# fpgasystems/GPU-FPGA-Recommendation-System

Measured on AMD Instinct MI355X. Metric: inferences/sec at batch 256, higher is better.
Workload: dtype f32; 1 GPU; Model-A (embedding_47_krnl: 47 tables, 1.415 GB) batch=256, fp32 FC 352-1024-512-256-1, all tables resident in one GPU's HBM; hash-filled tables, uniform per-table indices; index rows resident in HBM when the timed region starts (1024 rotating buffers), scores left in HBM (the bench contract's definition of `value`); value_pcie_inclusive = the reference's own loop (cuda_server.c:460-461,494-495): ; batch=256, driver_threads=2, workers_per_thread=2, batches_per_launch=64, parallelism=replicas x1

## Files before the change

gpu-fpga-recommendation-system_amd/csrc/fr_api.cpp:

```cpp
#include <chrono>
#include <cmath>
#include <cstdarg>
#include <cstdio>
#include <cstdlib>
#include <cstring>
#include <new>

#include "fr_internal.h"

static thread_local char g_err[512] = "";

void fr_set_error(const char *fmt, ...) {
    va_list ap;
    va_start(ap, fmt);
    vsnprintf(g_err, sizeof(g_err), fmt, ap);
    va_end(ap);
}

#ifdef FR_EXPERIMENTS
int fr_knob_env(const char *name, int dflt) {
    const char *e = getenv(name);
    return e ? atoi(e) : dflt;
}
#endif
// ... 718 lines not shown
    if (w->ctx) (void)hipSetDevice(w->ctx->device);
    fr_comm_worker_release(w);
    if (w->stream) (void)hipStreamSynchronize(w->stream);
    if (w->counted) w->ctx->n_workers.fetch_sub(1, std::memory_order_relaxed);
    if (w->h_idx) (void)hipHostFree(w->h_idx);
    if (w->h_pool_w) (void)hipHostFree(w->h_pool_w);
    if (w->h_pool_off) (void)hipHostFree(w->h_pool_off);
    if (w->h_dense) (void)hipHostFree(w->h_dense);
    if (w->h_score) (void)hipHostFree(w->h_score);
    if (w->h_err) (void)hipHostFree(w->h_err);
    if (w->h_sh_status) (void)hipHostFree(w->h_sh_status);
    if (w->h_stage_send) (void)hipHostFree(w->h_stage_send);
    if (w->h_stage_recv) (void)hipHostFree(w->h_stage_recv);
    void *dev[] = {w->d_idx, w->d_dense, w->d_records, w->d_act[0], w->d_act[1], w->d_score, w->d_slice, w->d_gathered, w->d_score_part, w->d_score_all};
    for (void *p : dev)
        if (p) (void)hipFree(p);
    if (w->hr.h_idx) (void)hipHostFree(w->hr.h_idx);
    if (w->hr.h_dense) (void)hipHostFree(w->hr.h_dense);
    if (w->hr.h_sc) (void)hipHostFree(w->hr.h_sc);
    void *hdev[] = {w->hr.d_idx, w->hr.d_dense, w->hr.d_sc};
    for (void *p : hdev)
        if (p) (void)hipFree(p);
    for (hipEvent_t e : w->hr.ev)
        if (e) (void)hipEventDestroy(e);
    for (hipEvent_t e : w->hr.ev_in)
        if (e) (void)hipEventDestroy(e);
    if (w->hr.copy) {
        (void)hipStreamSynchronize(w->hr.copy);
        (void)hipStreamDestroy(w->hr.copy);
    }
    if (w->h_blist) (void)hipHostFree(w->h_blist);
    if (w->d_blist) (void)hipFree(w->d_blist);
    for (hipEvent_t e : w->ev_blist)
        if (e) (void)hipEventDestroy(e);
    if (w->ev_update) (void)hipEventDestroy(w->ev_update);
    if (w->ev_start) (void)hipEventDestroy(w->ev_start);
    if (w->ev_stop) (void)hipEventDestroy(w->ev_stop);
    if (w->stream) (void)hipStreamDestroy(w->stream);
    fr_ctx *held = w->counted ? w->ctx : nullptr;
    delete w;
    fr_ctx_unref(held);
}

static size_t idx_cols(const fr_ctx *c) {
    const int mode = c->model.index_mode;
    return mode == FR_INDEX_PER_TABLE ? (size_t)c->model.n_tables : (mode == FR_INDEX_PER_BANK ? (size_t)c->n_banks : 1);
}

#define W_HIP(call)                                                                       \
    do {                                                                                  \
        hipError_t e_ = (call);                                                           \
        if (e_ != hipSuccess) {                                                           \
            fr_set_error("%s failed: %s", #call, hipGetErrorString(e_));                  \
            fr_worker_destroy(w);                                                         \
            return (e_ == hipErrorOutOfMemory) ? FR_ERR_OOM : FR_ERR_HIP;                 \
        }                                                                                 \
    } while (0)

extern "C" int fr_worker_create(fr_ctx *ctx, int max_batch, fr_worker **out) {
    if (!ctx || !out) FR_FAIL(FR_ERR_INVALID, "NULL argument");
    *out = nullptr;
    if (max_batch <= 0 || max_batch > (1 << 24)) FR_FAIL(FR_ERR_INVALID, "max_batch %d out of range", max_batch);
    {
        int widest = 0;
        for (int l = 0; l < 4; l++) widest = ctx->model.fc[l] > widest ? ctx->model.fc[l] : widest;
        if ((uint64_t)widest * (uint64_t)round_up(max_batch, 64) * 4ull >= (1ull << 32))
// ... 520 lines not shown
extern "C" int fr_ctx_set_small_block(fr_ctx *ctx, int max_batches) {
    if (!ctx) FR_FAIL(FR_ERR_INVALID, "ctx is NULL");
    if (max_batches < 0 || max_batches > 8) FR_FAIL(FR_ERR_INVALID, "max_batches %d outside [0, 8]", max_batches);
    ctx->small_block.store(max_batches, std::memory_order_relaxed);
    return FR_OK;
}

extern "C" int fr_ctx_stream_group(const fr_ctx *ctx) { return (ctx && !ctx->cpu && fused_eligible(ctx)) ? fused_group(ctx) : 1; }

static int fused_launch_slice(fr_worker *w, FrFusedArgs &a, int first, int n) {
    fr_ctx *c = w->ctx;
    const bool bf16 = c->fc_precision == FR_FC_BF16, fp8 = c->fc_precision == FR_FC_FP8;
    const int m2_forced = FR_KNOB_ONCE("FUSED_M2", -1);
    int tiles64 = 0;
    for (int i = 0; i < n; i++) tiles64 += (w->pending[first + i].batch + 63) / 64;
    const bool m2 = !bf16 && c->fc_precision == FR_FC_FP32 && frk_fused_m2_ok(c->model.fc[0], c->model.fc[1], c->model.fc[2], c->model.fc[3]) &&
                    (m2_forced == 1 || (m2_forced != 0 && fused_group(c) >= 64 && tiles64 > 128));
    const int per_wg = (bf16 || fp8) ? frk_fused_h_items_per_wg() : (m2 ? 64 : 32);
    int max_tiles = 0;
    for (int i = 0; i < n; i++) {
        a.b[i] = w->pending[first + i];
        const int tiles = (a.b[i].batch + per_wg - 1) / per_wg;
        if (tiles > max_tiles) max_tiles = tiles;
    }
    a.n_batches = n;
    a.tiles_per_batch = max_tiles;
    a.blist = nullptr;
    if (fp8) return frk_fused_f8_launch(a, w->stream);
    if (m2) return frk_fused_m2_launch(a, w->stream);
    if (bf16) return frk_fused_h_launch(a, w->stream);
    return frk_fused_launch(a, w->stream);
}

static int fused_flush(fr_worker *w) {
    if (w->n_pending == 0) return FR_OK;
    fr_ctx *c = w->ctx;
    FrFusedArgs a{};
    const bool bf16 = c->fc_precision == FR_FC_BF16, fp8 = c->fc_precision == FR_FC_FP8;
    a.words = c->d_words;
    a.n_words = c->n_words;
    a.idx_stride = (int)idx_cols(c);
    a.err_flag = w->d_err;
    if (fp8) {
        a.w1q = reinterpret_cast<const float4 *>(c->d_w_fp8[0]);
        a.w2q = reinterpret_cast<const float4 *>(c->d_w_fp8[1]);
        a.w3q = reinterpret_cast<const float4 *>(c->d_w_fp8[2]);
        a.wout = c->d_w[3];
        for (int l = 0; l < 3; l++) a.e_w[l] = c->f8_e_w[l];
        for (int l = 0; l < 4; l++) a.e_act[l] = c->f8_e_act[l];
    } else if (bf16) {
        a.w1q = reinterpret_cast<const float4 *>(c->d_w_bf16[0]);
        a.w2q = reinterpret_cast<const float4 *>(c->d_w_bf16[1]);
        a.w3q = reinterpret_cast<const float4 *>(c->d_w_bf16[2]);
        a.wout = reinterpret_cast<const float *>(c->d_w_bf16[3]);
    } else {
        a.w1q = reinterpret_cast<const float4 *>(c->d_wq[0]);
        a.w2q = reinterpret_cast<const float4 *>(c->d_wq[1]);
        a.w3q = reinterpret_cast<const float4 *>(c->d_wq[2]);
        a.wout = c->d_w[3];
    }
    a.K = c->model.fc[0];
    a.H1 = c->model.fc[1];
    a.H2 = c->model.fc[2];
    a.H3 = c->model.fc[3];
    a.stamps = g_stamp_buffer;
    const int n_all = w->n_pending;
    w->n_pending = 0;
    w->pending_items = 0;
    struct Keep {
        fr_worker *w;
        ~Keep() { keep_kernel(w); }
    } keep{w};
    if (bf16 || (fp8 && FR_KNOB_ONCE("FUSED_HK", -1) == 1 && c->d_w_fp8h[0] && c->d_w_fp8h[1] && c->d_w_fp8h[2])) {
        int tiles = 0, max_tiles = 0;
        for (int i = 0; i < n_all; i++) {
            const int t_ = (w->pending[i].batch + 63) / 64;
            tiles += t_;
            if (t_ > max_tiles) max_tiles = t_;
        }
        const int hk = FR_KNOB_ONCE("FUSED_HK", -1);
        const int hs_from = a.K <= 352 ? c->n_cu : c->n_cu + c->n_cu / 4;
        const bool only_hs = bf16 && !frk_fused_h_ok(a.K, a.H1, a.H2, a.H3);
        if (c->hk_ok == 1 && (only_hs || (hk != 0 && (hk == 1 || tiles >= hs_from)))) {
            if (!w->h_blist) {
                FR_HIP(hipHostMalloc((void **)&w->h_blist, sizeof(FrFusedBatch) * FR_FUSED_MAX_QUEUE * FR_BLIST_RING, hipHostMallocDefault));
                FR_HIP(hipMalloc((void **)&w->d_blist, sizeof(FrFusedBatch) * FR_FUSED_MAX_QUEUE * FR_BLIST_RING));
                for (int k = 0; k < FR_BLIST_RING; k++) FR_HIP(hipEventCreateWithFlags(&w->ev_blist[k], hipEventDisableTiming));
            }
            const int k = w->blist_cur;
            w->blist_cur = (k + 1) % FR_BLIST_RING;
            if (w->blist_busy[k]) FR_HIP(hipEventSynchronize(w->ev_blist[k]));
            FrFusedBatch *hb = w->h_blist + (size_t)k * FR_FUSED_MAX_QUEUE, *db = w->d_blist + (size_t)k * FR_FUSED_MAX_QUEUE;
            memcpy(hb, w->pending, sizeof(FrFusedBatch) * n_all);
            FR_HIP(hipMemcpyAsync(db, hb, sizeof(FrFusedBatch) * n_all, hipMemcpyHostToDevice, w->stream));
            FR_HIP(hipEventRecord(w->ev_blist[k], w->stream));
            w->blist_busy[k] = true;
            a.blist = db;
            a.n_batches = n_all;
            a.tiles_per_batch = max_tiles;
            if (bf16 && frk_fused_hk_takes_lp_rows(a.K) && lp_image_applies_hs(c)) {
                const int irc = lp_ensure_image(c, FR_FC_BF16);
                if (irc) return irc;
                a.words = c->d_words_lp;
                a.src_lp = 1;
            }
            if (bf16 && FR_KNOB_ONCE("FUSED_HS_ABLATE", 0)) a.e_act[3] = -776 - FR_KNOB_ONCE("FUSED_HS_ABLATE", 0);
            if (fp8) {
                a.w1q = reinterpret_cast<const float4 *>(c->d_w_fp8h[0]);
                a.w2q = reinterpret_cast<const float4 *>(c->d_w_fp8h[1]);
                a.w3q = reinterpret_cast<const float4 *>(c->d_w_fp8h[2]);
            }
            return frk_fused_hk_launch(a, c->n_cu, c->fc_precision, w->stream);
        }
    }
    for (int first = 0; first < n_all; first += FR_FUSED_MAX_BATCHES) {
        const int n = n_all - first < FR_FUSED_MAX_BATCHES ? n_all - first : FR_FUSED_MAX_BATCHES;
        int rc = fused_launch_slice(w, a, first, n);
        if (rc) return rc;
    }
    return FR_OK;
}

static int check_gather_args(fr_worker *w, const int32_t *d_idx, const float *d_dense) {
    fr_ctx *c = w->ctx;
    if (!d_idx) FR_FAIL(FR_ERR_INVALID, "d_idx is NULL");
    if (c->model.dense_len && !d_dense) FR_FAIL(FR_ERR_INVALID, "model has dense features but d_dense is NULL");
    return FR_OK;
}

static int launch_fc(fr_worker *w, int batch, const float *d_records, float *d_scores) {
    fr_ctx *c = w->ctx;
    if (c->n_shards > 1) FR_FAIL(FR_ERR_STATE, "fc on a sharded ctx needs the all-gathered records (use the sharded driver: fr_worker_submit_sharded, fr_worker_submit_sharded_pooled)");
    if (c->cpu) {
        frc_fc_chain(c->model.fc, c->d_w, d_records, batch, w->c_scratch, d_scores);
        return FR_OK;
    }
    if (w->n_active) FR_FAIL(FR_ERR_STATE, "pipeline busy: call fr_worker_sync first");
    if (w->launch_no == 0) w->launch_no = 1;
    const int ldm = round_up(batch, 32);
    const int par_prev = (int)((w->launch_no - 1) & 1);
    int rc;
    if (c->fc_precision == FR_FC_FP8) rc = frk_records_to_q16_fp8(d_records, act_set(w, par_prev).x, batch, c->model.fc[0], ldm, c->f8_e_act[0], w->stream);
    else if (c->fc_precision == FR_FC_BF16) rc = frk_records_to_q8_bf16(d_records, act_set(w, par_prev).x, batch, c->model.fc[0], ldm, w->stream);
    else rc = frk_transpose_records(d_records, act_set(w, par_prev).x, batch, c->model.fc[0], ldm, w->stream);
    if (rc) return rc;
    rc = pipeline_push(w, batch, 1, nullptr, nullptr, d_scores);
    if (rc) return rc;
    return pipeline_flush(w);
}

static int fc_from_slices_impl(fr_worker *w, int batch_total, int item0, int n_items, const float *d_gathered, float *d_scores, uint64_t *stage1_launch) {
    int rc = check_ready(w, n_items, false, true);
    if (rc) return rc;
// ... 464 lines not shown
    if (rc) return rc;
    if (!d_scores) FR_FAIL(FR_ERR_INVALID, "d_scores is NULL");
    fr_ctx *c = w->ctx;
    if (c->n_shards > 1 || c->model.layout != FR_LAYOUT_SEMANTIC)
        FR_FAIL(FR_ERR_STATE, "push_device needs an unsharded SEMANTIC-layout context");
    rc = check_gather_args(w, d_idx, d_dense);
    if (rc) return rc;
    if (c->cpu) {
        rc = launch_pipeline(w, batch, d_idx, d_dense, d_scores);
        if (rc) return rc;
        w->in_flight = true;
        return FR_OK;
    }
    FR_SET_DEVICE(c);
    const bool idx_fits = (size_t)batch * idx_cols(c) * sizeof(int32_t) < ((size_t)4000 << 20);
    const bool fused = fused_eligible(c) && fused_group(c) >= FR_FUSED_MIN_GROUP && idx_fits;
    if (fused && w->n_active > 0) {
        rc = pipeline_flush(w);
        if (rc) return rc;
    }
    if (!fused && w->n_pending > 0) {
        rc = fused_flush(w);
        if (rc) return rc;
    }
    if (fused) {
        FrFusedBatch &fb = w->pending[w->n_pending++];
        fb.idx = d_idx;
        fb.dense = d_dense;
        fb.scores = d_scores;
        fb.batch = batch;
        w->pending_items += batch;
        w->in_flight = true;
        const bool big = c->fc_precision == FR_FC_BF16 || (c->fc_precision == FR_FC_FP8 && FR_KNOB_ONCE("FUSED_HK", -1) == 1);
        const int64_t max_items = FR_KNOB_ONCE("FUSED_ITEMS", 0) ? FR_KNOB_ONCE("FUSED_ITEMS", 0) : (big ? 4096 * 64 : 256 * 64);
        return (w->n_pending >= fused_group(c) || w->pending_items >= max_items || w->n_pending >= FR_FUSED_MAX_QUEUE) ? fused_flush(w) : FR_OK;
    }
    rc = pipeline_push(w, batch, 0, d_idx, d_dense, d_scores);
    if (rc) return rc;
    w->in_flight = true;
    return FR_OK;
}

extern "C" int fr_worker_push_device_list(fr_worker *w, int n, const int *batch, const int32_t *const *d_idx, const float *const *d_dense,
                                          float *const *d_scores) {
    if (!w) FR_FAIL(FR_ERR_INVALID, "worker is NULL");
    if (n < 0 || (n > 0 && (!batch || !d_idx || !d_scores))) FR_FAIL(FR_ERR_INVALID, "push_device_list: n = %d needs batch, d_idx and d_scores arrays", n);
    for (int i = 0; i < n; i++) {
        const int rc = fr_worker_push_device(w, batch[i], d_idx[i], d_dense ? d_dense[i] : nullptr, d_scores[i]);
        if (rc) return rc;
    }
    return FR_OK;
}

static int push_pooled_impl(fr_worker *w, int batch, const int32_t *d_idx, const float *d_weights, const float *d_dense, float *d_scores, const int32_t *d_offsets = nullptr,
                            int64_t nnz = 0) {
    int rc = check_ready(w, batch, true, true);
    if (rc) return rc;
    if (!d_scores) FR_FAIL(FR_ERR_INVALID, "d_scores is NULL");
    fr_ctx *c = w->ctx;
    const bool weighted = d_weights != nullptr;
    if (c->pool_cols <= 0)
        FR_FAIL(FR_ERR_STATE, c->n_shards > 1 ? "no pooling is set on the sharded context: create it with fr_ctx_create_sharded_pooled" : "no pooling is set on the context: call fr_ctx_set_pooling first");
    if (c->n_shards > 1) FR_FAIL(FR_ERR_STATE, "a pooled push on a sharded ctx: the chain needs the all-gathered slices (fr_worker_submit_sharded_pooled)");
    if (c->model.layout != FR_LAYOUT_SEMANTIC) FR_FAIL(FR_ERR_STATE, "a pooled push needs a SEMANTIC-layout context");
    if (c->cpu) {
        rc = submit_pooled_impl(w, batch, d_idx, d_weights, weighted, d_dense, d_scores, d_offsets, nnz);
        if (rc) return rc;
        w->in_flight = true;
// ... 613 lines not shown
```

gpu-fpga-recommendation-system_amd/csrc/fr_fused.hip:

```cpp
#include "fr_device.h"

constexpr int FR_FT_LD = 33;

template <int NT, int D>
__device__ __forceinline__ void ft_load_a(float4 (&r)[D][NT], const float4 *__restrict__ aq, int N, int g) {
#pragma unroll
    for (int i = 0; i < D; i++)
#pragma unroll
        for (int t = 0; t < NT; t++) r[i][t] = aq[(size_t)(2 * (g + i)) * N + 32 * t];
}

template <int NT, int D>
__device__ __forceinline__ void ft_compute(f32x16 (&acc)[NT], f32x16 &alt, const float4 (&r)[D][NT], const uint4 *bl, int gb) {
    uint4 rb[D];
#pragma unroll
    for (int i = 0; i < D; i++) rb[i] = bl[(size_t)(2 * (gb + i)) * FR_FT_LD];
    __builtin_amdgcn_sched_barrier(0);
#pragma unroll
    for (int i = 0; i < D; i++) {
        const float bx = __uint_as_float(rb[i].x), by = __uint_as_float(rb[i].y), bz = __uint_as_float(rb[i].z), bw = __uint_as_float(rb[i].w);
        if constexpr (NT == 1) {
            acc[0] = __builtin_amdgcn_mfma_f32_32x32x2f32(r[i][0].x, bx, acc[0], 0, 0, 0);
            alt = __builtin_amdgcn_mfma_f32_32x32x2f32(r[i][0].y, by, alt, 0, 0, 0);
            acc[0] = __builtin_amdgcn_mfma_f32_32x32x2f32(r[i][0].z, bz, acc[0], 0, 0, 0);
// ... 394 lines not shown
    for (int g = 0; g < CNT; g++) {
        uint4 bnext[MT];
        const int gn = (g + 1 < CNT) ? g + 1 : g;
#pragma unroll
        for (int mt = 0; mt < MT; mt++) bnext[mt] = bl[(size_t)(2 * gn) * FR_M2_LD + 32 * mt];
        const float4(&a4)[NT] = ring[g % R];
#pragma unroll
        for (int c = 0; c < 4; c++)
#pragma unroll
            for (int t = 0; t < NT; t++)
#pragma unroll
                for (int mt = 0; mt < MT; mt++) {
                    const float av = c == 0 ? a4[t].x : c == 1 ? a4[t].y : c == 2 ? a4[t].z : a4[t].w;
                    const uint32_t bv = c == 0 ? bcur[mt].x : c == 1 ? bcur[mt].y : c == 2 ? bcur[mt].z : bcur[mt].w;
                    if (NT == 1 && (c & 1)) alt[mt] = __builtin_amdgcn_mfma_f32_32x32x2f32(av, __uint_as_float(bv), alt[mt], 0, 0, 0);
                    else acc[t][mt] = __builtin_amdgcn_mfma_f32_32x32x2f32(av, __uint_as_float(bv), acc[t][mt], 0, 0, 0);
                }
        if (g + R < CNT) {
#pragma unroll
            for (int t = 0; t < NT; t++) ring[g % R][t] = ft_wload(w, s0 + (unsigned)(g + R) * w.row2, 512 * t);
        }
        __builtin_amdgcn_sched_barrier(0);
#pragma unroll
        for (int mt = 0; mt < MT; mt++) bcur[mt] = bnext[mt];
    }
    if constexpr (NT == 1) {
#pragma unroll
        for (int mt = 0; mt < MT; mt++)
#pragma unroll
            for (int i = 0; i < 16; i++) acc[0][mt][i] += alt[mt][i];
    }
}

__device__ __forceinline__ void ftm_store_tile(uint4 *img, const f32x16 &acc, int n_local, int m_local, int hk, int lm) {
#pragma unroll
    for (int i = 0; i < 4; i++) {
        uint4 v;
        v.x = __float_as_uint(acc[4 * i + 0]);
        v.y = __float_as_uint(acc[4 * i + 1]);
        v.z = __float_as_uint(acc[4 * i + 2]);
        v.w = __float_as_uint(acc[4 * i + 3]);
        img[(size_t)((n_local >> 2) + 2 * i + hk) * FR_M2_LD + m_local + lm] = v;
    }
}

template <int KG>
__global__ void __launch_bounds__(512) fr_fused_tile_m2_kernel(const FrFusedArgs a) {
    extern __shared__ uint4 lds[];
    constexpr int LD = FR_M2_LD, MT = 2, T2W = 2, TI = 64;
    constexpr int RA = 12, RB = 8;
    const int KQ = a.K / 4;
    uint4 *Xq = lds;
    uint4 *R1 = Xq + (size_t)KQ * LD;
    uint4 *R2 = lds;
    uint4 *R3 = lds;
    const int tid = threadIdx.x, lane = tid & 63;
    const int wave = __builtin_amdgcn_readfirstlane(tid >> 6);
    const int hk = lane >> 5, lm = lane & 31;
    const int bi = blockIdx.x / a.tiles_per_batch, tile = blockIdx.x - bi * a.tiles_per_batch;
    const FrFusedBatch &bt = a.b[bi];
    const int m0 = tile * TI;
    if (m0 >= bt.batch) return;
    const FtW W1 = ft_w(a.w1q, a.K, a.H1, hk, lm), W2 = ft_w(a.w2q, a.H1, a.H2, hk, lm), W3 = ft_w(a.w3q, a.H2, a.H3, hk, lm);
    float4 ring1[RA][1];
    ft_ring_fill<1, RA, KG>(ring1, W1, 32 * wave, 0);

    {
        const int wl = tid & 63, ig = tid >> 6;
        constexpr int NB = (2 * KG + 63) / 64;
        const bool bad = ft_gather_tile<NB, 8>(a, bt, m0, wl, ig, [&](int w, int i, const uint4 &x) { Xq[(size_t)w * LD + 8 * ig + i] = x; });
        if (bad) atomicOr_system(a.err_flag, 1);
    }
    __syncthreads();

    f32x16 acc2[T2W][MT];
#pragma unroll
    for (int t = 0; t < T2W; t++)
#pragma unroll
        for (int mt = 0; mt < MT; mt++)
#pragma unroll
            for (int i = 0; i < 16; i++) acc2[t][mt][i] = 0.0f;
// ... 32 lines not shown
    ftm_gemm_ct<1, MT, RA, 32 * T2W>(acc3, ring3, W3, 32 * wave, R2, 0, 0, hk, lm);
    __syncthreads();
#pragma unroll
    for (int mt = 0; mt < MT; mt++) ftm_store_tile(R3, acc3[0][mt], 32 * wave, 32 * mt, hk, lm);
    __syncthreads();
    {
        const int il = tid & 63, sg = tid >> 6;
        const int rows_per = (a.H3 / 4) / 16;
        float *part = reinterpret_cast<float *>(R3 + (size_t)(a.H3 / 4) * LD);
#pragma unroll
        for (int h2 = 0; h2 < 2; h2++) {
            const int sl = 2 * sg + h2;
            float s = 0.0f;
            for (int q = sl * rows_per; q < (sl + 1) * rows_per; q++) {
                const uint4 r = R3[(size_t)q * LD + il];
                const float4 w4 = reinterpret_cast<const float4 *>(a.wout)[q];
                s = fmaf(w4.x, __uint_as_float(r.x), s);
                s = fmaf(w4.y, __uint_as_float(r.y), s);
                s = fmaf(w4.z, __uint_as_float(r.z), s);
                s = fmaf(w4.w, __uint_as_float(r.w), s);
            }
            part[sl * 64 + il] = s;
        }
        __syncthreads();
        if (tid < 64 && m0 + tid < bt.batch) {
            float t = part[tid];
#pragma unroll
            for (int i = 1; i < 16; i++) t += part[i * 64 + tid];
            bt.scores[m0 + tid] = t;
        }
    }
}

bool frk_fused_m2_ok(int K, int H1, int H2, int H3) { return K == 352 && H1 % 256 == 0 && H2 == 512 && H3 == 256; }

int frk_fused_m2_launch(const FrFusedArgs &a, hipStream_t s) {
    static FrLdsAttrOnce lds_once;
    if (int rc_ = fr_allow_full_lds(&fr_fused_tile_m2_kernel<44>, lds_once)) return rc_;
    const size_t rows1 = (size_t)(a.K / 4) + 64, rows2 = (size_t)(a.H2 / 4), rows3 = 64 + 4;
    const size_t rows = rows1 > rows2 ? (rows1 > rows3 ? rows1 : rows3) : (rows2 > rows3 ? rows2 : rows3);
    fr_fused_tile_m2_kernel<44><<<dim3(a.n_batches * a.tiles_per_batch), dim3(512), rows * FR_M2_LD * 16, s>>>(a);
    fr_note_kernel("fr_fused_tile_m2_kernel<44>");
    KCHECK();
    return FR_OK;
}

template <int NT, int MT, int R, int CNT>
__device__ __forceinline__ void fth_gemm_ct(f32x16 (&acc)[NT][MT], const FtW &w, int n0, const uint4 *Bh, int ld, int gb0, int g0, int hk, int lm) {
    const unsigned s0 = (unsigned)g0 * w.row2 + (unsigned)n0 * 16u;
    const uint4 *bl = Bh + (size_t)(2 * gb0 + hk) * ld + lm;
    uint4 ring[R][NT];
#pragma unroll
    for (int g = 0; g < R && g < CNT; g++)
#pragma unroll
        for (int t = 0; t < NT; t++) ring[g][t] = __builtin_bit_cast(uint4, ft_wload(w, s0 + (unsigned)g * w.row2, 512 * t));
#pragma unroll
    for (int g = 0; g < CNT; g++) {
        uint4 b8[MT];
#pragma unroll
        for (int mt = 0; mt < MT; mt++) b8[mt] = bl[(size_t)(2 * g) * ld + 32 * mt];
#pragma unroll
        for (int t = 0; t < NT; t++)
#pragma unroll
            for (int mt = 0; mt < MT; mt++)
                acc[t][mt] = __builtin_amdgcn_mfma_f32_32x32x16_bf16(__builtin_bit_cast(bf16x8, ring[g % R][t]), __builtin_bit_cast(bf16x8, b8[mt]),
                                                                     acc[t][mt], 0, 0, 0);
        if (g + R < CNT) {
#pragma unroll
            for (int t = 0; t < NT; t++) ring[g % R][t] = __builtin_bit_cast(uint4, ft_wload(w, s0 + (unsigned)(g + R) * w.row2, 512 * t));
        }
        __builtin_amdgcn_sched_barrier(0);
    }
}

// ... 406 lines not shown
```

gpu-fpga-recommendation-system_amd/csrc/fr_internal.h:

```cpp
#pragma once

#include <hip/hip_runtime.h>

#include <atomic>
#include <mutex>
#include <cstdint>
#include <string>
#include <vector>

#include "fleetrec.h"
#include "fleetrec_diag.h"
#include "fleetrec_serving.h"

void fr_set_error(const char *fmt, ...) __attribute__((format(printf, 1, 2)));

#define FR_FAIL(code, ...)         \
    do {                           \
        fr_set_error(__VA_ARGS__); \
        return (code);             \
    } while (0)

#define FR_HIP(call)                                                                                 \
    do {                                                                                             \
        hipError_t e_ = (call);                                                                      \
// ... 229 lines not shown
    int c_err = 0;
    double c_t0 = 0.0;
    hipStream_t stream = nullptr;
    int32_t *h_idx = nullptr;
    float *h_dense = nullptr;
    float *h_score = nullptr;
    int32_t *d_idx = nullptr;
    float *d_dense = nullptr;
    float *d_records = nullptr;
    float *d_act[2] = {nullptr, nullptr};
    int ld_max = 0;
    struct Slot {
        bool active = false;
        uint64_t launch0 = 0;
        int first_stage = 0;
        int batch = 0, ldm = 0;
        const int32_t *d_idx = nullptr;
        const float *d_dense = nullptr;
        float *d_scores = nullptr;
    } ring[8];
    uint64_t launch_no = 0;
    int n_active = 0;
    bool counted = false;
    bool diag_launch = false;
    bool calibrating = false;
    int last_x_parity = 0;
    FrFusedBatch pending[FR_FUSED_MAX_QUEUE];
    int n_pending = 0;
    FrFusedBatch *h_blist = nullptr, *d_blist = nullptr;
    hipEvent_t ev_blist[FR_BLIST_RING] = {nullptr, nullptr, nullptr, nullptr};
    bool blist_busy[FR_BLIST_RING] = {false, false, false, false};
    int blist_cur = 0;
    int64_t pending_items = 0;
    float *d_score = nullptr;
    struct HostRing {
        int g = 0;
        size_t idx_slot = 0, dense_slot = 0, score_slot = 0;
        int32_t *h_idx = nullptr, *d_idx = nullptr;
        float *h_dense = nullptr, *d_dense = nullptr, *h_sc = nullptr, *d_sc = nullptr;
        hipEvent_t ev[4] = {nullptr, nullptr, nullptr, nullptr};
        hipStream_t copy = nullptr;
        hipEvent_t ev_in[4] = {nullptr, nullptr, nullptr, nullptr};
        bool inflight[4] = {false, false, false, false};
        int count[4] = {0, 0, 0, 0};
        float *dst[4][FR_FUSED_MAX_BATCHES];
        int bsz[4][FR_FUSED_MAX_BATCHES];
        int cur = 0;
        int staged = 0;
        long long delivered = 0;
    } hr;
    void *d_slice = nullptr, *d_gathered = nullptr;
    float *d_score_part = nullptr, *d_score_all = nullptr;
    float *h_sh_status = nullptr;
    struct fr_comm *sh_comm = nullptr;
    int sh_ranks = 0;
    std::atomic<int> sh_inject_fc_fail{0};
    void *h_stage_send = nullptr, *h_stage_recv = nullptr;
    void *sh_host_stream = nullptr;
    int *h_err = nullptr;
    int *d_err = nullptr;
    bool in_flight = false;
    hipEvent_t ev_update = nullptr;
    bool update_recorded = false;
    char last_kernel[96] = "";
    hipEvent_t ev_start = nullptr, ev_stop = nullptr;
};
// ... 35 lines not shown
int frk_scatter_rows(float *head, int64_t row_stride_bytes, float *tail, int64_t head_rows, int64_t rows, int dim, int n, const int32_t *ids, const float *src, int *err_flag,
                     hipStream_t s);
int frk_gather(const FrWordDesc *words, int n_words, const FrGatherGroups &groups, const int32_t *idx, int idx_stride, const float *dense, void *out, int batch, int *err_flag,
               int transport, int e_x, hipStream_t s, int out_words, bool one_chunk = false);
int frk_gather_pooled(const FrWordDesc *words, const FrPoolDesc *pool, int n_words, const FrGatherGroups &groups, const int32_t *idx, const float *weights, int pool_cols,
                      int max_hots, bool wide, bool any_mean, const float *dense, void *out, int batch, int *err_flag, hipStream_t s, int out_words,
                      const int32_t *offsets = nullptr, int n_icols = 0, long long nnz = 0, int operand = 0, int ldm = 0, int e_x = 0, bool item_major = false);
int frk_gather_tile(const FrPassDesc *passes, const FrChunkDesc *chunks, int n_chunks, const int32_t *idx, int idx_stride, const float *dense, void *out,
                    int out_stride_words, int batch, int *err_flag, bool dedup, unsigned long long *dup_counter, hipStream_t s);
int frk_transpose_slices_lp(int precision, const void *gathered, int n_shards, int batch_total, int slice_padded, const int *h_offsets, const int *h_lens,
                            int item0, int n_items, void *X, int K, int ldm, hipStream_t s);
int frk_pipeline_launch(const FrPipeArgs &a, int single_stage, int precision, hipStream_t s);
int frk_pack_weights_q8_bf16(const float *W, uint16_t *Wh, int K, int H, hipStream_t s);
bool frk_fc_lp_gemm_ok(int precision, int K, int N, int ldm);
int frk_fc_lp_gemm(int precision, const void *Wp, const void *Xp, void *Yp, int K, int N, int ldm, int e_w, int e_in, int e_out, int width, bool minor, hipStream_t s);
bool frk_fused_hk_takes_lp_rows(int K);
bool frk_fc_tail_ok(int precision, int K, int N, int ldm);
int frk_fc_tail(int precision, const void *W3, const void *R2, const void *wout, float *scores, int K, int N, int ldm, int batch, int e_w, int e_in, int e_r3, hipStream_t s);
int frk_records_to_q8_bf16(const float *X, void *Xh, int batch, int K, int ldm, hipStream_t s);
int frk_pack_weights_q16_fp8(const float *W, void *Wf, int K, int H, int e_w, hipStream_t s);
int frk_pack_weights_q16h_fp8(const float *W, void *Wg, int K, int H, int e_w, hipStream_t s);
int frk_records_to_q16_fp8(const float *X, void *Xf, int batch, int K, int ldm, int e_x, hipStream_t s);
int frk_stats(const float *p, size_t n, void *d_out, hipStream_t s);
int frk_q4_to_lp(int precision, const float *Xq, void *Xo, int K, int ldm, int e_x, hipStream_t s);
int frk_stage_blocks_f8_gather(int K, int ldm);
int frk_pack_weights_q4(const float *W, float *Wq, int K, int H, hipStream_t s);
int frk_stage_blocks(int stage, int n_words, int K, int N, int ldm, int nsplit);
int frk_gather_tr_blocks(int n_words, int ldm, int variant);
int frk_gather_tr_variant(int batch, int idx_stride);
bool frk_fused_ok(int K, int H1, int H2, int H3);
int frk_fused_launch(const FrFusedArgs &a, hipStream_t s);
bool frk_fused_m2_ok(int K, int H1, int H2, int H3);
int frk_fused_m2_launch(const FrFusedArgs &a, hipStream_t s);
bool frk_fused_h_ok(int K, int H1, int H2, int H3);
bool frk_fused_f8_ok(int K, int H1, int H2, int H3);
int frk_fused_f8_launch(const FrFusedArgs &a, hipStream_t s);
int frk_fused_h_items_per_wg();
int frk_fused_h_launch(const FrFusedArgs &a, hipStream_t s);
bool frk_fused_hk_ok(int K, int H1, int H2, int H3, const FrWordDesc *h_words, int n_words);
int frk_fused_hk_launch(const FrFusedArgs &a, int n_cu, int precision, hipStream_t s);
int frk_transpose_records(const float *X, float *Xt, int batch, int K, int ldm, hipStream_t s);
int frk_transpose_slices(const float *gathered, int n_shards, int batch_total, int slice_padded, const int *h_offsets, const int *h_lens,
                         int item0, int n_items, float *Xq, int ldm, hipStream_t s);
void fr_shard_bounds(const fr_model_desc &m, int n_shards, std::vector<int> &seg_begin);
int fr_bank_map(const fr_model_desc &m, std::vector<int> &bank_of_table, std::vector<int64_t> &bank_min_rows);
```

Baseline: 69.31 million inferences/s.

## Add persistent fp32 fused MLP kernel overlapping next-tile gather with layer-3 GEMM

Adds a persistent variant of the fp32 m2 fused kernel that launches one workgroup per CU and loops over tiles taken from a device-resident batch list. Inside the layer-3 GEMM it issues the descriptor, index and embedding-row loads for the next tile through scheduling hooks, so gather latency hides behind MFMA work. The host side now holds pushes to enlarge launches, flushes only whole CU fills when it can, and uses events to detect a launch backlog. This removes per-tile workgroup launch and gather-stall costs, in exchange for more complex flush logic, extra latency from held batches and higher register pressure.

```diff
diff --git a/gpu-fpga-recommendation-system_amd/csrc/fr_api.cpp b/gpu-fpga-recommendation-system_amd/csrc/fr_api.cpp
--- a/gpu-fpga-recommendation-system_amd/csrc/fr_api.cpp
+++ b/gpu-fpga-recommendation-system_amd/csrc/fr_api.cpp
@@ -774,6 +774,8 @@
     if (w->h_blist) (void)hipHostFree(w->h_blist);
     if (w->d_blist) (void)hipFree(w->d_blist);
     for (hipEvent_t e : w->ev_blist)
+        if (e) (void)hipEventDestroy(e);
+    for (hipEvent_t e : w->ev_fused)
         if (e) (void)hipEventDestroy(e);
     if (w->ev_update) (void)hipEventDestroy(w->ev_update);
     if (w->ev_start) (void)hipEventDestroy(w->ev_start);
@@ -1360,8 +1362,30 @@
     return frk_fused_launch(a, w->stream);
 }
 
-static int fused_flush(fr_worker *w) {
-    if (w->n_pending == 0) return FR_OK;
+static bool fused_p32_persistent(const fr_ctx *c) {
+    return c->fc_precision == FR_FC_FP32 && c->n_cu > 0 && FR_KNOB_ONCE("FUSED_M2", -1) != 0 && fused_group(c) >= 64 &&
+           frk_fused_m2_ok(c->model.fc[0], c->model.fc[1], c->model.fc[2], c->model.fc[3]);
+}
+
+static int fused_stage_blist(fr_worker *w, int n, const FrFusedBatch **d_list) {
+    if (!w->h_blist) {
+        FR_HIP(hipHostMalloc((void **)&w->h_blist, sizeof(FrFusedBatch) * FR_FUSED_MAX_QUEUE * FR_BLIST_RING, hipHostMallocDefault));
+        FR_HIP(hipMalloc((void **)&w->d_blist, sizeof(FrFusedBatch) * FR_FUSED_MAX_QUEUE * FR_BLIST_RING));
+        for (int k = 0; k < FR_BLIST_RING; k++) FR_HIP(hipEventCreateWithFlags(&w->ev_blist[k], hipEventDisableTiming));
+    }
+    const int k = w->blist_cur;
+    w->blist_cur = (k + 1) % FR_BLIST_RING;
+    if (w->blist_busy[k]) FR_HIP(hipEventSynchronize(w->ev_blist[k]));
+    FrFusedBatch *hb = w->h_blist + (size_t)k * FR_FUSED_MAX_QUEUE, *db = w->d_blist + (size_t)k * FR_FUSED_MAX_QUEUE;
+    memcpy(hb, w->pending, sizeof(FrFusedBatch) * n);
+    FR_HIP(hipMemcpyAsync(db, hb, sizeof(FrFusedBatch) * n, hipMemcpyHostToDevice, w->stream));
+    FR_HIP(hipEventRecord(w->ev_blist[k], w->stream));
+    w->blist_busy[k] = true;
+    *d_list = db;
+    return FR_OK;
+}
+
+static int fused_launch_first(fr_worker *w, const int n_all) {
     fr_ctx *c = w->ctx;
     FrFusedArgs a{};
     const bool bf16 = c->fc_precision == FR_FC_BF16, fp8 = c->fc_precision == FR_FC_FP8;
@@ -1392,9 +1416,6 @@
     a.H2 = c->model.fc[2];
     a.H3 = c->model.fc[3];
     a.stamps = g_stamp_buffer;
-    const int n_all = w->n_pending;
-    w->n_pending = 0;
-    w->pending_items = 0;
     struct Keep {
         fr_worker *w;
         ~Keep() { keep_kernel(w); }
@@ -1410,20 +1431,7 @@
         const int hs_from = a.K <= 352 ? c->n_cu : c->n_cu + c->n_cu / 4;
         const bool only_hs = bf16 && !frk_fused_h_ok(a.K, a.H1, a.H2, a.H3);
         if (c->hk_ok == 1 && (only_hs || (hk != 0 && (hk == 1 || tiles >= hs_from)))) {
-            if (!w->h_blist) {
-                FR_HIP(hipHostMalloc((void **)&w->h_blist, sizeof(FrFusedBatch) * FR_FUSED_MAX_QUEUE * FR_BLIST_RING, hipHostMallocDefault));
-                FR_HIP(hipMalloc((void **)&w->d_blist, sizeof(FrFusedBatch) * FR_FUSED_MAX_QUEUE * FR_BLIST_RING));
-                for (int k = 0; k < FR_BLIST_RING; k++) FR_HIP(hipEventCreateWithFlags(&w->ev_blist[k], hipEventDisableTiming));
-            }
-            const int k = w->blist_cur;
-            w->blist_cur = (k + 1) % FR_BLIST_RING;
-            if (w->blist_busy[k]) FR_HIP(hipEventSynchronize(w->ev_blist[k]));
-            FrFusedBatch *hb = w->h_blist + (size_t)k * FR_FUSED_MAX_QUEUE, *db = w->d_blist + (size_t)k * FR_FUSED_MAX_QUEUE;
-            memcpy(hb, w->pending, sizeof(FrFusedBatch) * n_all);
-            FR_HIP(hipMemcpyAsync(db, hb, sizeof(FrFusedBatch) * n_all, hipMemcpyHostToDevice, w->stream));
-            FR_HIP(hipEventRecord(w->ev_blist[k], w->stream));
-            w->blist_busy[k] = true;
-            a.blist = db;
+            if (int rc_ = fused_stage_blist(w, n_all, &a.blist)) return rc_;
             a.n_batches = n_all;
             a.tiles_per_batch = max_tiles;
             if (bf16 && frk_fused_hk_takes_lp_rows(a.K) && lp_image_applies_hs(c)) {
@@ -1441,12 +1449,69 @@
             return frk_fused_hk_launch(a, c->n_cu, c->fc_precision, w->stream);
         }
     }
+    if (fused_p32_persistent(c)) {
+        int tiles = 0, max_tiles = 0;
+        for (int i = 0; i < n_all; i++) {
+            const int t_ = (w->pending[i].batch + 63) / 64;
+            tiles += t_;
+            if (t_ > max_tiles) max_tiles = t_;
+        }
+        const int from_pct = FR_KNOB_ONCE("FUSED_M2P_FROM", 100);
+        if (from_pct > 0 && (int64_t)tiles * 100 > (int64_t)c->n_cu * from_pct) {
+            if (int rc_ = fused_stage_blist(w, n_all, &a.blist)) return rc_;
+            a.n_batches = n_all;
+            a.tiles_per_batch = max_tiles;
+            return frk_fused_m2p_launch(a, c->n_cu, w->stream);
+        }
+    }
     for (int first = 0; first < n_all; first += FR_FUSED_MAX_BATCHES) {
         const int n = n_all - first < FR_FUSED_MAX_BATCHES ? n_all - first : FR_FUSED_MAX_BATCHES;
         int rc = fused_launch_slice(w, a, first, n);
         if (rc) return rc;
     }
     return FR_OK;
+}
+
+static int fused_flush(fr_worker *w, bool whole_fills = false, bool due_push = false) {
+    if (w->n_pending == 0) return FR_OK;
+    fr_ctx *c = w->ctx;
+    int n = w->n_pending;
+    if (whole_fills) {
+        int tiles = 0, best = 0;
+        for (int i = 0; i < w->n_pending; i++) {
+            tiles += (w->pending[i].batch + 63) / 64;
+            if (tiles % c->n_cu == 0) best = i + 1;
+        }
+        if (best > 0) n = best;
+    }
+    w->held_pushes = 0;
+    int rc = fused_launch_first(w, n);
+    if (rc == FR_OK && due_push && fused_p32_persistent(c)) {
+        hipEvent_t &ev = w->ev_fused[w->n_fused_launches % FR_BLIST_RING];
+        if (!ev && hipEventCreateWithFlags(&ev, hipEventDisableTiming) != hipSuccess) {
+            ev = nullptr;
+            rc = FR_ERR_HIP;
+            fr_set_error("hipEventCreate failed (fused launch event)");
+        } else if (hipEventRecord(ev, w->stream) != hipSuccess) {
+            rc = FR_ERR_HIP;
+            fr_set_error("hipEventRecord failed (fused launch event)");
+        } else {
+            w->n_fused_launches++;
+        }
+    }
+    const int rem = rc == FR_OK ? w->n_pending - n : 0;
+    if (rem > 0) memmove(w->pending, w->pending + n, sizeof(FrFusedBatch) * rem);
+    w->n_pending = rem;
+    w->pending_items = 0;
+    for (int i = 0; i < rem; i++) w->pending_items += w->pending[i].batch;
+    return rc;
+}
+
+static bool fused_backlogged(fr_worker *w) {
+    if (w->n_fused_launches < 2) return false;
+    if (hipEventQuery(w->ev_fused[(w->n_fused_launches - 2) % FR_BLIST_RING]) != hipErrorNotReady) return false;
+    (void)hipGetLastError();
+    return true;
 }
 
 static int check_gather_args(fr_worker *w, const int32_t *d_idx, const float *d_dense) {
@@ -1977,8 +2042,15 @@
         w->pending_items += batch;
         w->in_flight = true;
         const bool big = c->fc_precision == FR_FC_BF16 || (c->fc_precision == FR_FC_FP8 && FR_KNOB_ONCE("FUSED_HK", -1) == 1);
-        const int64_t max_items = FR_KNOB_ONCE("FUSED_ITEMS", 0) ? FR_KNOB_ONCE("FUSED_ITEMS", 0) : (big ? 4096 * 64 : 256 * 64);
-        return (w->n_pending >= fused_group(c) || w->pending_items >= max_items || w->n_pending >= FR_FUSED_MAX_QUEUE) ? fused_flush(w) : FR_OK;
+        const bool p32 = fused_p32_persistent(c);
+        const int64_t max_items = FR_KNOB_ONCE("FUSED_ITEMS", 0) ? FR_KNOB_ONCE("FUSED_ITEMS", 0) : (big ? 4096 * 64 : 256 * 64 * (p32 ? fused_group(c) / 64 : 1));
+        if (w->n_pending < fused_group(c) && w->pending_items < max_items && w->n_pending < FR_FUSED_MAX_QUEUE) return FR_OK;
+        if (p32 && w->n_pending < FR_FUSED_MAX_QUEUE && w->pending_items < 4 * 256 * 64 &&
+            (w->held_pushes % 32 != 0 || fused_backlogged(w))) {
+            w->held_pushes++;
+            return FR_OK;
+        }
+        return fused_flush(w, w->held_pushes > 0, true);
     }
     rc = pipeline_push(w, batch, 0, d_idx, d_dense, d_scores);
     if (rc) return rc;
diff --git a/gpu-fpga-recommendation-system_amd/csrc/fr_fused.hip b/gpu-fpga-recommendation-system_amd/csrc/fr_fused.hip
--- a/gpu-fpga-recommendation-system_amd/csrc/fr_fused.hip
+++ b/gpu-fpga-recommendation-system_amd/csrc/fr_fused.hip
@@ -450,6 +450,66 @@
     }
 }
 
+template <int NT, int MT, int R, int CNT, int GA, int GB, typename HookA, typename HookB, typename HookG>
+__device__ __forceinline__ void ftm_gemm_ct_hooks(f32x16 (&acc)[NT][MT], float4 (&ring)[R][NT], const FtW &w, int n0, const uint4 *Bq, int gb0, int g0, int hk,
+                                                  int lm, HookA &&hook_a, HookB &&hook_b, HookG &&hook_g) {
+    static_assert(0 <= GA && GA < GB && GB < CNT, "hooks sit behind distinct groups, in order");
+    const unsigned s0 = (unsigned)g0 * w.row2 + (unsigned)n0 * 16u;
+    const uint4 *bl = Bq + (size_t)(2 * gb0 + hk) * FR_M2_LD + lm;
+    uint4 bcur[MT];
+#pragma unroll
+    for (int mt = 0; mt < MT; mt++) bcur[mt] = bl[32 * mt];
+    f32x16 alt[MT];
+    if constexpr (NT == 1) {
+#pragma unroll
+        for (int mt = 0; mt < MT; mt++)
+#pragma unroll
+            for (int i = 0; i < 16; i++) alt[mt][i] = 0.0f;
+    }
+    auto group = [&](int g) __attribute__((always_inline)) {
+        uint4 bnext[MT];
+        const int gn = (g + 1 < CNT) ? g + 1 : g;
+#pragma unroll
+        for (int mt = 0; mt < MT; mt++) bnext[mt] = bl[(size_t)(2 * gn) * FR_M2_LD + 32 * mt];
+        const float4(&a4)[NT] = ring[g % R];
+#pragma unroll
+        for (int c = 0; c < 4; c++)
+#pragma unroll
+            for (int t = 0; t < NT; t++)
+#pragma unroll
+                for (int mt = 0; mt < MT; mt++) {
+                    const float av = c == 0 ? a4[t].x : c == 1 ? a4[t].y : c == 2 ? a4[t].z : a4[t].w;
+                    const uint32_t bv = c == 0 ? bcur[mt].x : c == 1 ? bcur[mt].y : c == 2 ? bcur[mt].z : bcur[mt].w;
+                    if (NT == 1 && (c & 1)) alt[mt] = __builtin_amdgcn_mfma_f32_32x32x2f32(av, __uint_as_float(bv), alt[mt], 0, 0, 0);
+                    else acc[t][mt] = __builtin_amdgcn_mfma_f32_32x32x2f32(av, __uint_as_float(bv), acc[t][mt], 0, 0, 0);
+                }
+        if (g + R < CNT) {
+#pragma unroll
+            for (int t = 0; t < NT; t++) ring[g % R][t] = ft_wload(w, s0 + (unsigned)(g + R) * w.row2, 512 * t);
+        }
+        if (g > GB) hook_g(g);
+        __builtin_amdgcn_sched_barrier(0);
+#pragma unroll
+        for (int mt = 0; mt < MT; mt++) bcur[mt] = bnext[mt];
+    };
+#pragma unroll
+    for (int g = 0; g <= GA; g++) group(g);
+    hook_a();
+    __builtin_amdgcn_sched_barrier(0);
+#pragma unroll
+    for (int g = GA + 1; g <= GB; g++) group(g);
+    hook_b();
+    __builtin_amdgcn_sched_barrier(0);
+#pragma unroll
+    for (int g = GB + 1; g < CNT; g++) group(g);
+    if constexpr (NT == 1) {
+#pragma unroll
+        for (int mt = 0; mt < MT; mt++)
+#pragma unroll
+            for (int i = 0; i < 16; i++) acc[0][mt][i] += alt[mt][i];
+    }
+}
+
 __device__ __forceinline__ void ftm_store_tile(uint4 *img, const f32x16 &acc, int n_local, int m_local, int hk, int lm) {
 #pragma unroll
     for (int i = 0; i < 4; i++) {
@@ -463,8 +523,7 @@
 }
 
 template <int KG>
-__global__ void __launch_bounds__(512) fr_fused_tile_m2_kernel(const FrFusedArgs a) {
-    extern __shared__ uint4 lds[];
+__device__ __forceinline__ void ftm_one_tile(const FrFusedArgs &a, uint4 *lds) {
     constexpr int LD = FR_M2_LD, MT = 2, T2W = 2, TI = 64;
     constexpr int RA = 12, RB = 8;
     const int KQ = a.K / 4;
@@ -563,6 +622,209 @@
     }
 }
 
+template <int KG>
+__device__ __forceinline__ void ftm_persistent(const FrFusedArgs &a, uint4 *lds) {
+    constexpr int LD = FR_M2_LD, MT = 2, T2W = 2, TI = 64;
+    constexpr int RA = 12, RB = 8;
+    constexpr int G_DESC = 2, G_IDX = 9, G_ROW0 = 16, G_STEP = 3;
+    static_assert(2 * KG > 64 && 2 * KG <= 96, "the next-tile gather covers 65 .. 96 record words");
+    const int KQ = a.K / 4;
+    uint4 *Xq = lds;
+    uint4 *R1 = Xq + (size_t)KQ * LD;
+    uint4 *R2 = lds;
+    uint4 *R3 = R1;
+    float *part = reinterpret_cast<float *>(R1 + (size_t)64 * LD);
+    const int tid = threadIdx.x, lane = tid & 63;
+    const int wave = __builtin_amdgcn_readfirstlane(tid >> 6);
+    const int hk = lane >> 5, lm = lane & 31;
+    const int n_tiles = a.n_batches * a.tiles_per_batch;
+    typedef const FrFusedBatch __attribute__((address_space(4))) *blist_t;
+    const blist_t bl = (blist_t)a.blist;
+    auto batch_at = [&](int bi) {
+        FrFusedBatch r;
+        r.idx = bl[bi].idx, r.dense = bl[bi].dense, r.scores = bl[bi].scores, r.batch = bl[bi].batch, r.pad_ = 0;
+        return r;
+    };
+    auto next_tile = [&](int t) {
+        for (t += gridDim.x; t < n_tiles; t += gridDim.x) {
+            const int bi = t / a.tiles_per_batch;
+            if ((t - bi * a.tiles_per_batch) * TI < bl[bi].batch) break;
+        }
+        return t;
+    };
+    int t_cur = next_tile((int)blockIdx.x - (int)gridDim.x);
+    if (t_cur >= n_tiles) return;
+    auto tid_again = [&]() __attribute__((always_inline)) {
+        unsigned z = 0;
+        asm volatile("" : "+v"(z));
+        return (int)(64u * (unsigned)wave + __builtin_amdgcn_mbcnt_hi(~0u, __builtin_amdgcn_mbcnt_lo(~0u, z)));
+    };
+    const FtW W1 = ft_w(a.w1q, a.K, a.H1, hk, lm), W2 = ft_w(a.w2q, a.H1, a.H2, hk, lm), W3 = ft_w(a.w3q, a.H2, a.H3, hk, lm);
+    float4 ring1[RA][1];
+    ft_ring_fill<1, RA, KG>(ring1, W1, 32 * wave, 0);
+
+    {
+        const int bi = t_cur / a.tiles_per_batch;
+        const FrFusedBatch bt = batch_at(bi);
+        constexpr int NB = (2 * KG + 63) / 64;
+        const bool bad = ft_gather_tile<NB, 8>(a, bt, (t_cur - bi * a.tiles_per_batch) * TI, tid & 63, tid >> 6,
+                                               [&](int w, int i, const uint4 &x) { Xq[(size_t)w * LD + 8 * (tid >> 6) + i] = x; });
+        if (bad) atomicOr_system(a.err_flag, 1);
+    }
+    __syncthreads();
+
+    for (;;) {
+        f32x16 acc2[T2W][MT];
+#pragma unroll
+        for (int t = 0; t < T2W; t++)
+#pragma unroll
+            for (int mt = 0; mt < MT; mt++)
+#pragma unroll
+                for (int i = 0; i < 16; i++) acc2[t][mt][i] = 0.0f;
+        const int n_chunks = a.H1 / 256;
+        for (int c = 0; c < n_chunks; c++) {
+            f32x16 acc1[1][MT];
+#pragma unroll
+            for (int mt = 0; mt < MT; mt++)
+#pragma unroll
+                for (int i = 0; i < 16; i++) acc1[0][mt][i] = 0.0f;
+            ftm_gemm_ct<1, MT, RA, KG>(acc1, ring1, W1, c * 256 + 32 * wave, Xq, 0, 0, hk, lm);
+            float4 ring2[RB][T2W];
+            ft_ring_fill<T2W, RB, 32>(ring2, W2, 32 * T2W * wave, 32 * c);
+            if (c > 0) __syncthreads();
+#pragma unroll
+            for (int mt = 0; mt < MT; mt++) ftm_store_tile(R1, acc1[0][mt], 32 * wave, 32 * mt, hk, lm);
+            __syncthreads();
+            ftm_gemm_ct<T2W, MT, RB, 32>(acc2, ring2, W2, 32 * T2W * wave, R1, 0, 32 * c, hk, lm);
+            const int cn = (c + 1 < n_chunks) ? c + 1 : c;
+            ft_ring_fill<1, RA, KG>(ring1, W1, cn * 256 + 32 * wave, 0);
+        }
+        const int t_nxt = next_tile(t_cur);
+        const bool has_next = t_nxt < n_tiles;
+        const int t_g = has_next ? t_nxt : t_cur;
+        const int bi_g = t_g / a.tiles_per_batch;
+        const int m0_g = (t_g - bi_g * a.tiles_per_batch) * TI;
+        const FrFusedBatch bt_g = batch_at(bi_g);
+        const int32_t *const idx_g = bt_g.idx;
+        const float *const dense_g = bt_g.dense;
+        const int batch_g = bt_g.batch;
+        float4 ring3[RA][1];
+        ft_ring_fill<1, RA, 32 * T2W>(ring3, W3, 32 * wave, 0);
+        __syncthreads();
+#pragma unroll
+        for (int t = 0; t < T2W; t++)
+#pragma unroll
+            for (int mt = 0; mt < MT; mt++) ftm_store_tile(R2, acc2[t][mt], 32 * (T2W * wave + t), 32 * mt, hk, lm);
+        __syncthreads();
+
+        const int tg = tid_again();
+        const int gw[2] = {tg & 63, 64 + (tg & 31)};
+        const int gi[2] = {8 * (tg >> 6), 4 * (tg >> 5)};
+        uint4 g_d0[2];
+        uint32_t g_rows[2];
+        uint32_t g_id[12];
+        uint4 g_v[12];
+        bool g_bad = false;
+        const __amdgpu_buffer_rsrc_t rs_idx = __builtin_amdgcn_make_buffer_rsrc(const_cast<int32_t *>(idx_g), 0, (unsigned)batch_g * (unsigned)a.idx_stride * 4u, 0x00020000);
+        auto gather_desc = [&]() __attribute__((always_inline)) {
+            uint64_t wa = reinterpret_cast<uintptr_t>(a.words);
+            asm volatile("" : "+s"(wa));
+            typedef const u32x4_t __attribute__((address_space(1))) * gptr_t;
+            typedef const uint32_t __attribute__((address_space(1))) * gptr1_t;
+#pragma unroll
+            for (int p = 0; p < 2; p++) {
+                const int w = gw[p] < a.n_words ? gw[p] : a.n_words - 1;
+                const u32x4_t q = *(gptr_t)(wa + 32ull * (unsigned)w);
+                g_d0[p] = make_uint4(q.x, q.y, q.z, q.w);
+                g_rows[p] = *(gptr1_t)(wa + 32ull * (unsigned)w + 16);
+            }
+        };
+        auto gather_idx = [&]() __attribute__((always_inline)) {
+#pragma unroll
+            for (int j = 0; j < 12; j++) {
+                const int p = j < 8 ? 0 : 1, i = j < 8 ? j : j - 8;
+                const uint32_t icol = (g_d0[p].w & FR_DESC_DENSE) ? 0u : g_d0[p].w * 4u;
+                g_id[j] = (uint32_t)__builtin_amdgcn_raw_buffer_load_b32(rs_idx, (unsigned)(m0_g + gi[p] + i) * (unsigned)a.idx_stride * 4u + icol, 0, 0);
+            }
+        };
+        auto gather_rows = [&](int g) __attribute__((always_inline)) {
+            const int j = (g - G_ROW0) / G_STEP;
+            if (g >= G_ROW0 && (g - G_ROW0) % G_STEP == 0 && j < 12) {
+                const int p = j < 8 ? 0 : 1, i = j < 8 ? j : j - 8;
+                const bool dense = (g_d0[p].w & FR_DESC_DENSE) != 0;
+                const uint64_t base = (dense ? (uint64_t)reinterpret_cast<uintptr_t>(dense_g) : 0ull) + (((uint64_t)g_d0[p].y << 32) | g_d0[p].x);
+                const unsigned m = (unsigned)(m0_g + gi[p] + i);
+                uint32_t r = g_id[j];
+                const bool oob = !dense & (r >= g_rows[p]);
+                g_bad |= oob;
+                r = oob ? 0u : r;
+                r = dense ? (m < (unsigned)batch_g ? m : 0u) : r;
+                typedef const u32x4_t __attribute__((address_space(1))) * gptr_t;
+                const u32x4_t q = *(gptr_t)(base + (uint64_t)r * g_d0[p].z);
+                g_v[j] = make_uint4(q.x, q.y, q.z, q.w);
+            }
+        };
+        f32x16 acc3[1][MT];
+#pragma unroll
+        for (int mt = 0; mt < MT; mt++)
+#pragma unroll
+            for (int i = 0; i < 16; i++) acc3[0][mt][i] = 0.0f;
+        ftm_gemm_ct_hooks<1, MT, RA, 32 * T2W, G_DESC, G_IDX>(acc3, ring3, W3, 32 * wave, R2, 0, 0, hk, lm, gather_desc, gather_idx, gather_rows);
+        __syncthreads();
+        ft_ring_fill<1, RA, KG>(ring1, W1, 32 * wave, 0);
+#pragma unroll
+        for (int mt = 0; mt < MT; mt++) ftm_store_tile(R3, acc3[0][mt], 32 * wave, 32 * mt, hk, lm);
+        if (has_next) {
+#pragma unroll
+            for (int j = 0; j < 12; j++) {
+                const int p = j < 8 ? 0 : 1, i = j < 8 ? j : j - 8;
+                if (gw[p] < a.n_words) Xq[(size_t)gw[p] * LD + gi[p] + i] = (m0_g + gi[p] + i < batch_g) ? g_v[j] : make_uint4(0u, 0u, 0u, 0u);
+            }
+            if (g_bad) atomicOr_system(a.err_flag, 1);
+        }
+        __syncthreads();
+        {
+            const int bi = t_cur / a.tiles_per_batch;
+            const int m0 = (t_cur - bi * a.tiles_per_batch) * TI;
+            float *const scores = bl[bi].scores;
+            const int batch = bl[bi].batch;
+            const int te = tid_again();
+            const int il = te & 63, sg = te >> 6;
+            const int rows_per = (a.H3 / 4) / 16;
+#pragma unroll
+            for (int h2 = 0; h2 < 2; h2++) {
+                const int sl = 2 * sg + h2;
+                float s = 0.0f;
+                for (int q = sl * rows_per; q < (sl + 1) * rows_per; q++) {
+                    const uint4 r = R3[(size_t)q * LD + il];
+                    const float4 w4 = reinterpret_cast<const float4 *>(a.wout)[q];
+                    s = fmaf(w4.x, __uint_as_float(r.x), s);
+                    s = fmaf(w4.y, __uint_as_float(r.y), s);
+                    s = fmaf(w4.z, __uint_as_float(r.z), s);
+                    s = fmaf(w4.w, __uint_as_float(r.w), s);
+                }
+                part[sl * 64 + il] = s;
+            }
+            __syncthreads();
+            if (te < 64 && m0 + te < batch) {
+                float t = part[te];
+#pragma unroll
+                for (int i = 1; i < 16; i++) t += part[i * 64 + te];
+                scores[m0 + te] = t;
+            }
+        }
+        if (!has_next) break;
+        t_cur = t_nxt;
+    }
+}
+
+template <int KG>
+__global__ void __launch_bounds__(512) fr_fused_tile_m2_kernel(const FrFusedArgs a) {
+    extern __shared__ uint4 lds[];
+    if (a.blist) ftm_persistent<KG>(a, lds);
+    else ftm_one_tile<KG>(a, lds);
+}
+
 bool frk_fused_m2_ok(int K, int H1, int H2, int H3) { return K == 352 && H1 % 256 == 0 && H2 == 512 && H3 == 256; }
 
 int frk_fused_m2_launch(const FrFusedArgs &a, hipStream_t s) {
@@ -571,6 +833,18 @@
     const size_t rows1 = (size_t)(a.K / 4) + 64, rows2 = (size_t)(a.H2 / 4), rows3 = 64 + 4;
     const size_t rows = rows1 > rows2 ? (rows1 > rows3 ? rows1 : rows3) : (rows2 > rows3 ? rows2 : rows3);
     fr_fused_tile_m2_kernel<44><<<dim3(a.n_batches * a.tiles_per_batch), dim3(512), rows * FR_M2_LD * 16, s>>>(a);
+    fr_note_kernel("fr_fused_tile_m2_kernel<44>");
+    KCHECK();
+    return FR_OK;
+}
+
+int frk_fused_m2p_launch(const FrFusedArgs &a, int n_cu, hipStream_t s) {
+    static FrLdsAttrOnce lds_once;
+    if (!a.blist) FR_FAIL(FR_ERR_INVALID, "internal: the persistent fp32 launch needs its batch list in device memory");
+    if (int rc_ = fr_allow_full_lds(&fr_fused_tile_m2_kernel<44>, lds_once)) return rc_;
+    const size_t rows1 = (size_t)(a.K / 4) + 64 + 4, rows2 = (size_t)(a.H2 / 4);
+    const int tiles = a.n_batches * a.tiles_per_batch;
+    fr_fused_tile_m2_kernel<44><<<dim3(tiles < n_cu ? tiles : n_cu), dim3(512), (rows1 > rows2 ? rows1 : rows2) * FR_M2_LD * 16, s>>>(a);
     fr_note_kernel("fr_fused_tile_m2_kernel<44>");
     KCHECK();
     return FR_OK;
diff --git a/gpu-fpga-recommendation-system_amd/csrc/fr_internal.h b/gpu-fpga-recommendation-system_amd/csrc/fr_internal.h
--- a/gpu-fpga-recommendation-system_amd/csrc/fr_internal.h
+++ b/gpu-fpga-recommendation-system_amd/csrc/fr_internal.h
@@ -285,6 +285,9 @@
     bool blist_busy[FR_BLIST_RING] = {false, false, false, false};
     int blist_cur = 0;
     int64_t pending_items = 0;
+    hipEvent_t ev_fused[FR_BLIST_RING] = {nullptr, nullptr, nullptr, nullptr};
+    int64_t n_fused_launches = 0;
+    int held_pushes = 0;
     float *d_score = nullptr;
     struct HostRing {
         int g = 0;
@@ -386,6 +389,7 @@
 int frk_fused_launch(const FrFusedArgs &a, hipStream_t s);
 bool frk_fused_m2_ok(int K, int H1, int H2, int H3);
 int frk_fused_m2_launch(const FrFusedArgs &a, hipStream_t s);
+int frk_fused_m2p_launch(const FrFusedArgs &a, int n_cu, hipStream_t s);
 bool frk_fused_h_ok(int K, int H1, int H2, int H3);
 bool frk_fused_f8_ok(int K, int H1, int H2, int H3);
 int frk_fused_f8_launch(const FrFusedArgs &a, hipStream_t s);
```

Measured after the change: 67.15 million inferences/s. -3.1%, worse.
